# sohmandal/classpose

Hardware: AMD Instinct MI355X
Metric: wsi_tiles_per_sec (higher is better)
Workload: dtype bf16; 1 GPU; configs[1]: synthetic 10000x10000 WSI (1936 tiles), tile 256 / overlap 32, conic 7 classes, ViT-L ClassTransformer depth 24 random-init, batch 32 sub-tiles = 8 WSI tiles/step, every step a distinct batch of the rank's shard (tiles sharded k % n_gpus, at most 256 distinct batches resident, longer runs wrap) streamed pinned host -> hipMemcpyAsync inside the timed region (the reader decodes ahead int; slide=10000, tile=256, overlap=32, batch_subtiles=32, distinct_batches=143, records_gathered=2048, decode_ahead_batches_at_t0=4, device_resident_batches_at_t0=1

## Files before the change

### classpose_amd/csrc/cpx_net.hip

```cpp
#include "cpx_internal.h"
#include <algorithm>

typedef __attribute__((ext_vector_type(8))) __bf16 bf16x8;
typedef __attribute__((ext_vector_type(8))) _Float16 f16x8;
typedef __attribute__((ext_vector_type(16))) float f32x16;

template <bool F16>
__device__ __forceinline__ f32x16 mfma32(const uint4 &a, const uint4 &b, f32x16 c) {
    if constexpr (F16)
        return __builtin_amdgcn_mfma_f32_32x32x16_f16(*reinterpret_cast<const f16x8 *>(&a),
                                                      *reinterpret_cast<const f16x8 *>(&b), c, 0, 0, 0);
    else
        return __builtin_amdgcn_mfma_f32_32x32x16_bf16(*reinterpret_cast<const bf16x8 *>(&a),
                                                       *reinterpret_cast<const bf16x8 *>(&b), c, 0, 0, 0);
}
template <bool F16>
__device__ __forceinline__ unsigned short h_from_f32(float f) {
    if constexpr (F16) { _Float16 h = (_Float16)f; return *reinterpret_cast<unsigned short *>(&h); }
    else return f32_to_bf16(f);
}
template <bool F16>
__device__ __forceinline__ float f32_from_h(unsigned short u) {
    if constexpr (F16) return (float)*reinterpret_cast<_Float16 *>(&u);
    else return bf16_to_f32(u);
}

typedef __attribute__((ext_vector_type(2))) float f32x2_t;
typedef __attribute__((ext_vector_type(2))) __bf16 bf16x2_t;
typedef __attribute__((ext_vector_type(2))) _Float16 f16x2_t;
template <bool F16>
__device__ __forceinline__ unsigned pack2(float lo, float hi) {
    f32x2_t v = {lo, hi};
    if constexpr (F16) return __builtin_bit_cast(unsigned, __builtin_convertvector(v, f16x2_t));
    else return __builtin_bit_cast(unsigned, __builtin_convertvector(v, bf16x2_t));
}

template <int C, bool F16>
__global__ void __launch_bounds__(256) k_layernorm(const unsigned short *__restrict__ x,
                                                   const float *__restrict__ w,
                                                   const float *__restrict__ b, int rows, float eps,
                                                   unsigned short *__restrict__ out) {
    constexpr int PER = C / 64;
    const int lane = threadIdx.x & 63;
    const int row = blockIdx.x * 4 + (threadIdx.x >> 6);
    if (row >= rows) return;
    const unsigned short *xr = x + (size_t)row * C + lane * PER;
    float v[PER];
    if constexpr (PER == 16) {
        uint4 a = *reinterpret_cast<const uint4 *>(xr), c = *reinterpret_cast<const uint4 *>(xr + 8);
        unsigned u[8] = {a.x, a.y, a.z, a.w, c.x, c.y, c.z, c.w};
#pragma unroll
        for (int i = 0; i < 8; ++i) { v[2 * i] = f32_from_h<F16>(u[i] & 0xFFFF); v[2 * i + 1] = f32_from_h<F16>(u[i] >> 16); }
    } else {
        uint2 a = *reinterpret_cast<const uint2 *>(xr);
        v[0] = f32_from_h<F16>(a.x & 0xFFFF); v[1] = f32_from_h<F16>(a.x >> 16);
        v[2] = f32_from_h<F16>(a.y & 0xFFFF); v[3] = f32_from_h<F16>(a.y >> 16);
    }
    float s = 0.f;
#pragma unroll
    for (int i = 0; i < PER; ++i) s += v[i];
#pragma unroll
    for (int o = 32; o > 0; o >>= 1) s += __shfl_xor(s, o);
    const float mean = s * (1.0f / C);
    float q = 0.f;
#pragma unroll
    for (int i = 0; i < PER; ++i) { float d = v[i] - mean; q += d * d; }
#pragma unroll
    for (int o = 32; o > 0; o >>= 1) q += __shfl_xor(q, o);
    const float rstd = rsqrtf(q * (1.0f / C) + eps);
    unsigned short o16[PER];
#pragma unroll
    for (int i = 0; i < PER; ++i) {
        float y = (v[i] - mean) * rstd * w[lane * PER + i] + b[lane * PER + i];
        o16[i] = h_from_f32<F16>(y);
    }
    unsigned short *orow = out + (size_t)row * C + lane * PER;
    if constexpr (PER == 16) {
        uint4 a, c;
        a.x = o16[0] | (o16[1] << 16); a.y = o16[2] | (o16[3] << 16); a.z = o16[4] | (o16[5] << 16); a.w = o16[6] | (o16[7] << 16);
        c.x = o16[8] | (o16[9] << 16); c.y = o16[10] | (o16[11] << 16); c.z = o16[12] | (o16[13] << 16); c.w = o16[14] | (o16[15] << 16);
        *reinterpret_cast<uint4 *>(orow) = a;
        *reinterpret_cast<uint4 *>(orow + 8) = c;
    } else {
        uint2 a;
        a.x = o16[0] | (o16[1] << 16); a.y = o16[2] | (o16[3] << 16);
        *reinterpret_cast<uint2 *>(orow) = a;
    }
}

int cpx_layernorm_half(int dtype, const void *x, const float *w, const float *b, int rows, int C,
                       float eps, void *out, void *stream) {
    CPX_REQUIRE(x && w && b && out && rows > 0 && (C == 1024 || C == 256));
    CPX_REQUIRE(dtype == CPX_DT_BF16 || dtype == CPX_DT_F16);
    hipStream_t s = (hipStream_t)stream;
    dim3 grid(cpx_cdiv(rows, 4)), block(256);
    const bool f16 = dtype == CPX_DT_F16;
    if (C == 1024) {
        if (f16) hipLaunchKernelGGL((k_layernorm<1024, true>), grid, block, 0, s, (const unsigned short *)x, w, b, rows, eps, (unsigned short *)out);
        else hipLaunchKernelGGL((k_layernorm<1024, false>), grid, block, 0, s, (const unsigned short *)x, w, b, rows, eps, (unsigned short *)out);
    } else {
        if (f16) hipLaunchKernelGGL((k_layernorm<256, true>), grid, block, 0, s, (const unsigned short *)x, w, b, rows, eps, (unsigned short *)out);
        else hipLaunchKernelGGL((k_layernorm<256, false>), grid, block, 0, s, (const unsigned short *)x, w, b, rows, eps, (unsigned short *)out);
    }
    CPX_CHECK_LAUNCH();
    return CPX_OK;
}
extern "C" int cpx_layernorm(int dtype, const void *x, const float *w, const float *b, int rows, int C,
                             float eps, void *out, void *stream) {
    if (dtype == CPX_DT_F32) return cpx_layernorm_f32((const float *)x, w, b, rows, C, eps, (float *)out, stream);
    return cpx_layernorm_half(dtype, x, w, b, rows, C, eps, out, stream);
}
extern "C" int cpx_layernorm_bf16(const void *x, const float *w, const float *b, int rows, int C,
                                  float eps, void *out, void *stream) {
    return cpx_layernorm_half(CPX_DT_BF16, x, w, b, rows, C, eps, out, stream);
}

__global__ void __launch_bounds__(256) k_v_transpose(const unsigned short *__restrict__ qkv,
                                                     unsigned short *__restrict__ vT) {
    __shared__ unsigned short tile[64][66];
    const int t0 = blockIdx.x * 64, h = blockIdx.y, s = blockIdx.z;
    const int tid = threadIdx.x;
    {
        int tok = tid >> 2, c = (tid & 3) * 16;
        const unsigned short *src = qkv + ((size_t)s * 1024 + t0 + tok) * 3072 + 2048 + h * 64 + c;
        uint4 a = *reinterpret_cast<const uint4 *>(src), b = *reinterpret_cast<const uint4 *>(src + 8);
        unsigned u[8] = {a.x, a.y, a.z, a.w, b.x, b.y, b.z, b.w};
#pragma unroll
        for (int i = 0; i < 8; ++i) { tile[tok][c + 2 * i] = u[i] & 0xFFFF; tile[tok][c + 2 * i + 1] = u[i] >> 16; }
    }
    __syncthreads();
    {
        int d = tid >> 2, c = (tid & 3) * 16;
        unsigned u[8];
#pragma unroll
        for (int i = 0; i < 8; ++i) u[i] = tile[c + 2 * i][d] | ((unsigned)tile[c + 2 * i + 1][d] << 16);
        unsigned short *dst = vT + (((size_t)s * 16 + h) * 64 + d) * 1024 + t0 + c;
        *reinterpret_cast<uint4 *>(dst) = make_uint4(u[0], u[1], u[2], u[3]);
        *reinterpret_cast<uint4 *>(dst + 8) = make_uint4(u[4], u[5], u[6], u[7]);
    }
}

#define ATT_THREADS 256
__device__ __forceinline__ int pi_perm(int r) { return (r & ~12) | ((r & 4) << 1) | ((r & 8) >> 1); }

#define A4_SLOT 8192
#define A4_G_LD 66
#define A4_LDS_BYTES (4 * A4_SLOT + 4 * 32 * A4_G_LD * 2)
template <int OFF>
__device__ __forceinline__ uint4 a4_read128(unsigned addr) {
    uint4 v;
    asm volatile("ds_read_b128 %0, %1 offset:%2" : "=v"(v) : "v"(addr), "n"(OFF));
    return v;
}
template <bool F16>
__global__ void __launch_bounds__(ATT_THREADS, 3) k_attention4p(const unsigned short *__restrict__ qkv,
                                                                const unsigned short *__restrict__ vT,
                                                                const unsigned short *__restrict__ relh,
                                                                const unsigned short *__restrict__ relw,
                                                                unsigned short *__restrict__ out, int xcd_order) {
    extern __shared__ __attribute__((aligned(16))) char a4_smem[];
    const int tid = threadIdx.x, lane = tid & 63;
    const int wave = __builtin_amdgcn_readfirstlane(tid >> 6);
    const int r = lane & 31, h2 = lane >> 5;
    const int lin = (blockIdx.z * gridDim.y + blockIdx.y) * gridDim.x + blockIdx.x;
    int rg = blockIdx.x, head = blockIdx.y, s = blockIdx.z;
    if (xcd_order) {
        const int j = lin >> 3, pair = (j >> 3) * 8 + (lin & 7);
        rg = j & 7; head = pair & 15; s = pair >> 4;
    }
    const int qh = rg * 4 + wave;
    const size_t tok0 = (size_t)s * 1024;
    const int kkey = tid >> 3, vd = tid >> 2;
    const unsigned short *ksrc = qkv + (tok0 + kkey) * 3072 + 1024 + head * 64 + (((tid & 7) ^ ((kkey >> 1) & 7)) * 8);
    const unsigned short *vsrc = vT + (((size_t)s * 16 + head) * 64 + vd) * 1024 + (((tid & 3) ^ ((vd >> 2) & 3)) * 8);
    char *dma_dst = a4_smem + wave * 1024;
    auto issue = [&](int kh) {
        char *d = dma_dst + (kh & 3) * A4_SLOT;
        __builtin_amdgcn_global_load_lds((const __attribute__((address_space(1))) void *)(ksrc + (size_t)kh * 32 * 3072),
                                         (__attribute__((address_space(3))) void *)d, 16, 0, 0);
        __builtin_amdgcn_global_load_lds((const __attribute__((address_space(1))) void *)(vsrc + kh * 32),
                                         (__attribute__((address_space(3))) void *)(d + 4096), 16, 0, 0);
    };
    issue(0); issue(1); issue(2);

    const unsigned short *qrow = qkv + (tok0 + qh * 32 + r) * 3072 + head * 64;
    uint4 qf[4];
#pragma unroll
    for (int ks = 0; ks < 4; ++ks) qf[ks] = *reinterpret_cast<const uint4 *>(qrow + 16 * ks + 8 * h2);
    _Float16 *G = reinterpret_cast<_Float16 *>(a4_smem + 4 * A4_SLOT) + wave * 32 * A4_G_LD;
    auto compute_G = [&](const unsigned short *table) {
#pragma unroll
        for (int jb = 0; jb < 2; ++jb) {
            f32x16 acc;
#pragma unroll
            for (int i = 0; i < 16; ++i) acc[i] = 0.f;
#pragma unroll
            for (int ks = 0; ks < 4; ++ks) {
                uint4 tf = *reinterpret_cast<const uint4 *>(table + (jb * 32 + r) * 64 + 16 * ks + 8 * h2);
                acc = mfma32<F16>(tf, qf[ks], acc);
            }
#pragma unroll
            for (int i = 0; i < 16; ++i) G[r * A4_G_LD + jb * 32 + (i & 3) + 8 * (i >> 2) + 4 * h2] = (_Float16)acc[i];
        }
    };
    compute_G(relw);
    f32x16 GW;
#pragma unroll
    for (int i = 0; i < 16; ++i) GW[i] = (float)G[r * A4_G_LD + (r - pi_perm((i & 3) + 8 * (i >> 2) + 4 * h2) + 31)];
    compute_G(relh);
    asm volatile("s_waitcnt vmcnt(0) lgkmcnt(0)" ::: "memory");
    __builtin_amdgcn_s_barrier();

    const unsigned lds0 = (unsigned)(size_t)(__attribute__((address_space(3))) char *)a4_smem;
    const int krow = pi_perm(r);
    unsigned ka[4], va[4];
#pragma unroll
    for (int ks = 0; ks < 4; ++ks) ka[ks] = lds0 + (unsigned)(krow * 128 + (((2 * ks + h2) ^ ((krow >> 1) & 7)) * 16));
#pragma unroll
    for (int db = 0; db < 2; ++db)
#pragma unroll
        for (int st = 0; st < 2; ++st) {
            const int d = db * 32 + r;
            va[db * 2 + st] = lds0 + 4096u + (unsigned)(d * 64 + (((2 * st + h2) ^ ((d >> 2) & 3)) * 16));
        }
    const unsigned gaddr = lds0 + 4u * A4_SLOT + (unsigned)((wave * 32 * A4_G_LD + r * A4_G_LD + qh + 31) * 2);

    auto qk = [&](auto slot_tag) {
        constexpr int SL = decltype(slot_tag)::value;
        const uint4 k0 = a4_read128<SL * A4_SLOT>(ka[0]), k1 = a4_read128<SL * A4_SLOT>(ka[1]);
        const uint4 k2 = a4_read128<SL * A4_SLOT>(ka[2]), k3 = a4_read128<SL * A4_SLOT>(ka[3]);
        asm volatile("s_waitcnt lgkmcnt(0)" ::: "memory");
        __builtin_amdgcn_sched_barrier(0);
        f32x16 S = mfma32<F16>(k0, qf[0], GW);
        S = mfma32<F16>(k1, qf[1], S);
        S = mfma32<F16>(k2, qf[2], S);
        S = mfma32<F16>(k3, qf[3], S);
        return S;
    };
    using std::integral_constant;
    f32x16 S = qk(integral_constant<int, 0>{});
    f32x16 O0, O1;
#pragma unroll
    for (int i = 0; i < 16; ++i) { O0[i] = 0.f; O1[i] = 0.f; }
    float m_run = -1e30f, l_run = 0.f;
    const float cexp = 0.125f * 1.44269504088896340736f;
    constexpr float HEADROOM = F16 ? 3.0f : 6.0f;

    auto tile = [&](const int kh, auto slot_tag, auto next_tag, auto tail_tag) {
        constexpr int SL = decltype(slot_tag)::value, SN = decltype(next_tag)::value, TAIL = decltype(tail_tag)::value;
        if constexpr (TAIL < 2) asm volatile("s_waitcnt vmcnt(2)" ::: "memory");
        else asm volatile("s_waitcnt vmcnt(0)" ::: "memory");
        __builtin_amdgcn_s_barrier();
        if constexpr (TAIL == 0) issue(kh + 3);
        unsigned gh_bits;
        asm volatile("ds_read_u16 %0, %1" : "=v"(gh_bits) : "v"(gaddr - 2u * (unsigned)kh));
        f32x16 Sn = S;
        if constexpr (TAIL < 3) Sn = qk(integral_constant<int, SN>{});
        else {
            asm volatile("s_waitcnt lgkmcnt(0)" : "+v"(gh_bits)::"memory");
            __builtin_amdgcn_sched_barrier(0);
        }
        const float gh = (float)__builtin_bit_cast(_Float16, (unsigned short)gh_bits);
        float p[16];
        unsigned pk[8];
        {
            const float off = (gh - m_run) * cexp;
#pragma unroll
            for (int i = 0; i < 16; ++i) p[i] = __builtin_amdgcn_exp2f(__builtin_fmaf(S[i], cexp, off));
#pragma unroll
            for (int j = 0; j < 8; ++j) pk[j] = pack2<F16>(p[2 * j], p[2 * j + 1]);
        }
        const bool resc = __builtin_expect(__any(((pk[0] | pk[1] | pk[2]) | (pk[3] | pk[4] | pk[5]) | (pk[6] | pk[7])) & 0x40004000u), 0);
        if (resc) {
            float mx = __builtin_fmaxf(__builtin_fmaxf(S[0], S[1]), S[2]);
#pragma unroll
            for (int i = 3; i < 15; i += 2) mx = __builtin_fmaxf(__builtin_fmaxf(mx, S[i]), S[i + 1]);
            mx = __builtin_fmaxf(mx, S[15]);
            mx = __builtin_fmaxf(mx, __shfl_xor(mx, 32)) + gh + HEADROOM / cexp;
            const float m_new = __builtin_fmaxf(m_run, mx);
            const float alpha = __builtin_amdgcn_exp2f((m_run - m_new) * cexp);
            m_run = m_new;
            l_run *= alpha;
#pragma unroll
            for (int i = 0; i < 16; ++i) { O0[i] *= alpha; O1[i] *= alpha; }
            const float off = (gh - m_run) * cexp;
#pragma unroll
            for (int i = 0; i < 16; ++i) p[i] = __builtin_amdgcn_exp2f(__builtin_fmaf(S[i], cexp, off));
#pragma unroll
            for (int j = 0; j < 8; ++j) pk[j] = pack2<F16>(p[2 * j], p[2 * j + 1]);
        }
        const float a0 = (p[0] + p[1]) + (p[2] + p[3]), a1 = (p[4] + p[5]) + (p[6] + p[7]);
        const float a2 = (p[8] + p[9]) + (p[10] + p[11]), a3 = (p[12] + p[13]) + (p[14] + p[15]);
        l_run += (a0 + a1) + (a2 + a3);
        const uint4 pf0 = make_uint4(pk[0], pk[1], pk[2], pk[3]), pf1 = make_uint4(pk[4], pk[5], pk[6], pk[7]);
        const uint4 v00 = a4_read128<SL * A4_SLOT>(va[0]), v01 = a4_read128<SL * A4_SLOT>(va[1]);
        const uint4 v10 = a4_read128<SL * A4_SLOT>(va[2]), v11 = a4_read128<SL * A4_SLOT>(va[3]);
        asm volatile("s_waitcnt lgkmcnt(0)" ::: "memory");
        __builtin_amdgcn_sched_barrier(0);
        O0 = mfma32<F16>(v00, pf0, O0);
        O1 = mfma32<F16>(v10, pf0, O1);
        O0 = mfma32<F16>(v01, pf1, O0);
        O1 = mfma32<F16>(v11, pf1, O1);
        S = Sn;
    };
    using T0 = integral_constant<int, 0>;
    for (int kh0 = 0; kh0 < 28; kh0 += 4) {
        tile(kh0 + 0, integral_constant<int, 0>{}, integral_constant<int, 1>{}, T0{});
        tile(kh0 + 1, integral_constant<int, 1>{}, integral_constant<int, 2>{}, T0{});
        tile(kh0 + 2, integral_constant<int, 2>{}, integral_constant<int, 3>{}, T0{});
        tile(kh0 + 3, integral_constant<int, 3>{}, integral_constant<int, 0>{}, T0{});
    }
    tile(28, integral_constant<int, 0>{}, integral_constant<int, 1>{}, T0{});
    tile(29, integral_constant<int, 1>{}, integral_constant<int, 2>{}, integral_constant<int, 1>{});
    tile(30, integral_constant<int, 2>{}, integral_constant<int, 3>{}, integral_constant<int, 2>{});
    tile(31, integral_constant<int, 3>{}, integral_constant<int, 0>{}, integral_constant<int, 3>{});
    const float inv = 1.0f / (l_run + __shfl_xor(l_run, 32));
    unsigned short *orow = out + (tok0 + qh * 32 + r) * 1024 + head * 64;
#pragma unroll
    for (int db = 0; db < 2; ++db)
#pragma unroll
        for (int g4 = 0; g4 < 4; g4 += 2) {
            const f32x16 &O = db ? O1 : O0;
            unsigned ax = pack2<F16>(O[4 * g4 + 0] * inv, O[4 * g4 + 1] * inv), ay = pack2<F16>(O[4 * g4 + 2] * inv, O[4 * g4 + 3] * inv);
            unsigned bx = pack2<F16>(O[4 * g4 + 4] * inv, O[4 * g4 + 5] * inv), by = pack2<F16>(O[4 * g4 + 6] * inv, O[4 * g4 + 7] * inv);
            const auto rx = __builtin_amdgcn_permlane32_swap(ax, bx, false, false);
            const auto ry = __builtin_amdgcn_permlane32_swap(ay, by, false, false);
            *reinterpret_cast<uint4 *>(orow + db * 32 + 8 * g4 + 8 * h2) = make_uint4(rx[0], ry[0], rx[1], ry[1]);
        }
}

CPX_SWITCH(g_att_xcd, 1);
CPX_SWITCH(g_att_v8, 2);
#ifdef CPX_DEBUG
extern "C" void cpx_attention_set_variant(int v8) { g_att_v8 = v8; }
extern "C" void cpx_attention_set_xcd_order(int v) { g_att_xcd = v; }
#endif
extern "C" int cpx_attention_relpos(const void *qkv, const void *rel_h, const void *rel_w,
                                    int n_subtiles, void *vT_ws, void *out, void *stream) {
    return cpx_attention_half(CPX_DT_BF16, qkv, rel_h, rel_w, n_subtiles, vT_ws, out, stream, true);
}
extern "C" int cpx_attention(int dtype, const void *qkv, const void *rel_h, const void *rel_w,
                             int n_subtiles, void *vT_ws, void *out, void *stream) {
    if (dtype == CPX_DT_F32)
        return cpx_attention_f32((const float *)qkv, (const float *)rel_h, (const float *)rel_w, n_subtiles, (float *)out, stream);
    return cpx_attention_half(dtype, qkv, rel_h, rel_w, n_subtiles, vT_ws, out, stream, true);
}
int cpx_attention_half(int dtype, const void *qkv, const void *rel_h, const void *rel_w, int n_subtiles,
                       void *vT_ws, void *out, void *stream, bool transpose_v) {
    CPX_REQUIRE(qkv && rel_h && rel_w && vT_ws && out && n_subtiles > 0);
    CPX_REQUIRE(dtype == CPX_DT_BF16 || dtype == CPX_DT_F16);
#ifdef CPX_DEBUG
    CPX_REQUIRE(g_att_v8 == 2 || g_att_v8 == 7);
#endif
    hipStream_t s = (hipStream_t)stream;
    if (transpose_v)
        hipLaunchKernelGGL(k_v_transpose, dim3(16, 16, n_subtiles), dim3(256), 0, s,
                           (const unsigned short *)qkv, (unsigned short *)vT_ws);
#ifdef CPX_DEBUG
    if (g_att_v8 == 7) {
        const dim3 grid4(8, 16, n_subtiles);
        static CpxOncePerDevice once4;
        once4([] {
            (void)hipFuncSetAttribute((const void *)k_attention4p<true>, hipFuncAttributeMaxDynamicSharedMemorySize, A4_LDS_BYTES);
            (void)hipFuncSetAttribute((const void *)k_attention4p<false>, hipFuncAttributeMaxDynamicSharedMemorySize, A4_LDS_BYTES);
        });
        if (dtype == CPX_DT_F16)
            hipLaunchKernelGGL((k_attention4p<true>), grid4, dim3(ATT_THREADS), A4_LDS_BYTES, s, (const unsigned short *)qkv, (const unsigned short *)vT_ws,
                               (const unsigned short *)rel_h, (const unsigned short *)rel_w, (unsigned short *)out, g_att_xcd);
        else
            hipLaunchKernelGGL((k_attention4p<false>), grid4, dim3(ATT_THREADS), A4_LDS_BYTES, s, (const unsigned short *)qkv, (const unsigned short *)vT_ws,
                               (const unsigned short *)rel_h, (const unsigned short *)rel_w, (unsigned short *)out, g_att_xcd);
        CPX_CHECK_LAUNCH();
        return CPX_OK;
    }
#endif
    return cpx_attention2w_launch(dtype, qkv, vT_ws, rel_h, rel_w, n_subtiles, out, g_att_xcd, s);
}

struct NetWs {
    size_t off_x, off_xn, off_qkv, off_vt, off_ao, off_h, off_neck, off_neck2, off_st, total;
};
static NetWs net_ws(int nS) {
    NetWs w; size_t o = 0; const size_t M = (size_t)nS * 1024;
    auto take = [&](size_t b) { size_t r = o; o = cpx_align_up(o + b, 256); return r; };
    w.off_x = take(M * 1024 * 2);
    w.off_xn = take(M * 1024 * 2);
    w.off_qkv = take(M * 3072 * 2);
    w.off_vt = take(M * 1024 * 2);
    w.off_ao = take(M * 1024 * 2);
    w.off_h = take(M * 4096 * 2);
    w.off_neck = take(M * 256 * 2);
    w.off_neck2 = take(M * 256 * 2);
    w.off_st = take(M * 8 * sizeof(float));
    w.total = o;
    return w;
}
extern "C" size_t cpx_net_workspace_bytes(int n_subtiles, int dtype) {
    if (n_subtiles <= 0) return 0;
    return dtype == CPX_DT_F32 ? cpx_net_f32_workspace_bytes(n_subtiles) : net_ws(n_subtiles).total;
}

extern "C" size_t cpx_net_neck_offset(int n_subtiles, int dtype) {
    if (n_subtiles <= 0 || dtype < CPX_DT_BF16 || dtype > CPX_DT_F32) return 0;
    return dtype == CPX_DT_F32 ? cpx_net_f32_neck_offset(n_subtiles) : net_ws(n_subtiles).off_neck2;
}
// ... 326 lines not shown
```

### classpose_amd/csrc/cpx_pre.hip

```cpp
#include "cpx_common.h"

#define NTHR 256

__device__ __forceinline__ void cv_linear_tap(int d, double scale, int slen, bool clamp_weight,
                                              int &s0, int &s1, int &w0, int &w1) {
    float f = (float)(((double)d + 0.5) * scale - 0.5);
    int s = (int)floorf(f);
    f -= (float)s;
    if (clamp_weight) {
        if (s < 0) { f = 0.f; s = 0; }
        if (s >= slen - 1) { f = 0.f; s = slen - 1; }
    }
    w0 = __float2int_rn((1.f - f) * 2048.f);
    w1 = __float2int_rn(f * 2048.f);
    s0 = min(max(s, 0), slen - 1);
    s1 = min(max(s + 1, 0), slen - 1);
}

__global__ void k_resize_linear_u8(const uint8_t *__restrict__ src, int sh, int sw,
                                   uint8_t *__restrict__ dst, int dh, int dw, double scale_x,
                                   double scale_y, int area2) {
    int p = blockIdx.x * NTHR + threadIdx.x;
    if (p >= dh * dw) return;
    int dy = p / dw, dx = p - dy * dw;
    const uint8_t *s = src + (size_t)blockIdx.y * sh * sw * 3;
    uint8_t *o = dst + ((size_t)blockIdx.y * dh * dw + p) * 3;
    if (area2) {
        const uint8_t *r0 = s + ((size_t)(2 * dy) * sw + 2 * dx) * 3, *r1 = r0 + (size_t)sw * 3;
        for (int c = 0; c < 3; ++c) o[c] = (uint8_t)((r0[c] + r0[3 + c] + r1[c] + r1[3 + c] + 2) >> 2);
        return;
    }
    int x0, x1, a0, a1, y0, y1, b0, b1;
    cv_linear_tap(dx, scale_x, sw, true, x0, x1, a0, a1);
    cv_linear_tap(dy, scale_y, sh, false, y0, y1, b0, b1);
    const uint8_t *r0 = s + (size_t)y0 * sw * 3, *r1 = s + (size_t)y1 * sw * 3;
    for (int c = 0; c < 3; ++c) {
        int h0 = r0[x0 * 3 + c] * a0 + r0[x1 * 3 + c] * a1;
        int h1 = r1[x0 * 3 + c] * a0 + r1[x1 * 3 + c] * a1;
        o[c] = (uint8_t)((((b0 * (h0 >> 4)) >> 16) + ((b1 * (h1 >> 4)) >> 16) + 2) >> 2);
    }
}

extern "C" int cpx_resize_linear_u8(const uint8_t *src, int nT, int sh, int sw, uint8_t *dst, int dh,
                                    int dw, void *stream) {
    CPX_REQUIRE(src && dst && nT > 0 && sh > 0 && sw > 0 && dh > 0 && dw > 0);
    CPX_REQUIRE((long long)dh * dw < (1ll << 31) && (long long)sh * sw < (1ll << 31));
    hipStream_t s = (hipStream_t)stream;
    if (sh == dh && sw == dw) {
        hipError_t e = hipMemcpyAsync(dst, src, (size_t)nT * sh * sw * 3, hipMemcpyDeviceToDevice, s);
        CPX_REQUIRE(e == hipSuccess);
        return CPX_OK;
    }
    double scale_x = 1.0 / ((double)dw / (double)sw), scale_y = 1.0 / ((double)dh / (double)sh);
    int area2 = (sw == 2 * dw && sh == 2 * dh) ? 1 : 0;
    hipLaunchKernelGGL(k_resize_linear_u8, dim3(cpx_cdiv((long long)dh * dw, NTHR), nT), dim3(NTHR), 0, s,
                       src, sh, sw, dst, dh, dw, scale_x, scale_y, area2);
    CPX_CHECK_LAUNCH();
    return CPX_OK;
}

__global__ void k_hist_u8(const uint8_t *__restrict__ tiles, int HW, uint32_t *__restrict__ hist) {
    __shared__ uint32_t sh[3 * 256];
    for (int i = threadIdx.x; i < 768; i += NTHR) sh[i] = 0;
    __syncthreads();
    const uint8_t *t = tiles + (size_t)blockIdx.y * HW * 3;
    for (int p = (blockIdx.x * NTHR + threadIdx.x) * 4; p < HW; p += gridDim.x * NTHR * 4) {
        int n = min(4, HW - p);
        for (int k = 0; k < n; ++k) {
            const uint8_t *px = t + (size_t)(p + k) * 3;
            atomicAdd(&sh[px[0]], 1u);
            atomicAdd(&sh[256 + px[1]], 1u);
            atomicAdd(&sh[512 + px[2]], 1u);
        }
    }
    __syncthreads();
    uint32_t *h = hist + (size_t)blockIdx.y * 768;
    for (int i = threadIdx.x; i < 768; i += NTHR)
        if (sh[i]) atomicAdd(&h[i], sh[i]);
}

__device__ __forceinline__ float np_lerp(float a, float b, float t) {
    float diff = b - a;
    float r = a + diff * t;
    if (t >= 0.5f) r = b - diff * (1.0f - t);
    return r;
}
__global__ void k_norm_stats(const uint32_t *__restrict__ hist, int nTC, int HW, int lo_prev,
                             float lo_g, int hi_prev, float hi_g, float *__restrict__ stats) {
    const int lane = threadIdx.x & 63;
    const int tc = (blockIdx.x * blockDim.x + threadIdx.x) >> 6;
    if (tc >= nTC) return;
    const uint4 c = *reinterpret_cast<const uint4 *>(hist + (size_t)tc * 256 + 4 * lane);
    const long long s0 = c.x, s1 = s0 + c.y, s2 = s1 + c.z, s3 = s2 + c.w;
    long long incl = s3;
#pragma unroll
    for (int o = 1; o < 64; o <<= 1) {
        const long long up = __shfl_up(incl, o);
        if (lane >= o) incl += up;
    }
    const long long excl = incl - s3;
    auto value_at = [&](int k) -> float {
        const unsigned long long m = __ballot(incl > (long long)k);
        const int l = __ffsll((long long)m) - 1;
        int v = 0;
        if (lane == l) v = 4 * lane + (excl + s0 > k ? 0 : (excl + s1 > k ? 1 : (excl + s2 > k ? 2 : 3)));
        return (float)__shfl(v, l);
    };
    const float g0 = value_at(lo_prev), g1 = value_at(min(lo_prev + 1, HW - 1));
    const float g2 = value_at(hi_prev), g3 = value_at(min(hi_prev + 1, HW - 1));
    const unsigned long long nz = __ballot(s3 > 0);
    const int lmin = __ffsll((long long)nz) - 1, lmax = 63 - __clzll((long long)nz);
    int vlo = 0, vhi = 0;
    if (lane == lmin) vlo = 4 * lane + (c.x ? 0 : (c.y ? 1 : (c.z ? 2 : 3)));
    if (lane == lmax) vhi = 4 * lane + (c.w ? 3 : (c.z ? 2 : (c.y ? 1 : 0)));
    const int vmin = __shfl(vlo, lmin), vmax = __shfl(vhi, lmax);
    if (lane != 0) return;
    float x01 = np_lerp(g0, g1, lo_g);
    float x99 = np_lerp(g2, g3, hi_g);
    float den = x99 - x01;
    float mode;
    if (vmax == vmin) mode = 0.f;
    else if (den > (float)1e-3) mode = 1.f;
    else mode = 2.f;
    stats[tc * 4 + 0] = x01;
    stats[tc * 4 + 1] = den;
    stats[tc * 4 + 2] = mode;
    stats[tc * 4 + 3] = x99;
}

__device__ __forceinline__ float norm_px(uint8_t v, const float *st) {
    float x = (float)v;
    float mode = st[2];
    if (mode == 1.f) { x = x - st[0]; x = __fdiv_rn(x, st[1]); }
    else if (mode == 2.f) x = 0.f;
    return x;
}

__global__ void k_norm_apply(const uint8_t *__restrict__ tiles, const float *__restrict__ stats,
                             int HW, float *__restrict__ out) {
    int i = blockIdx.x * NTHR + threadIdx.x;
    if (i >= HW * 3) return;
    size_t t = blockIdx.y;
    int c = i % 3;
    out[t * HW * 3 + i] = norm_px(tiles[t * HW * 3 + i], stats + (t * 3 + c) * 4);
}

extern "C" int cpx_normalize_stats_u8(const uint8_t *tiles, int nT, int H, int W, int lo_prev,
                                      float lo_gamma, int hi_prev, float hi_gamma, float *stats,
                                      uint32_t *hist_ws, void *stream) {
    CPX_REQUIRE(tiles && stats && hist_ws && nT > 0 && H > 0 && W > 0);
    CPX_REQUIRE(lo_prev >= 0 && hi_prev >= lo_prev && hi_prev < H * W);
    hipStream_t s = (hipStream_t)stream;
    CPX_HIP(hipMemsetAsync(hist_ws, 0, sizeof(uint32_t) * 768 * (size_t)nT, s));
    int nb = min(64, cpx_cdiv((long long)H * W, NTHR * 4));
    hipLaunchKernelGGL(k_hist_u8, dim3(nb, nT), dim3(NTHR), 0, s, tiles, H * W, hist_ws);
    hipLaunchKernelGGL(k_norm_stats, dim3(cpx_cdiv(nT * 3, 4)), dim3(256), 0, s, hist_ws, nT * 3,
                       H * W, lo_prev, lo_gamma, hi_prev, hi_gamma, stats);
    CPX_CHECK_LAUNCH();
    return CPX_OK;
}

extern "C" int cpx_normalize_apply_u8(const uint8_t *tiles, const float *stats, int nT, int H, int W,
                                      float *out, void *stream) {
    CPX_REQUIRE(tiles && stats && out && nT > 0 && H > 0 && W > 0);
    hipLaunchKernelGGL(k_norm_apply, dim3(cpx_cdiv((long long)H * W * 3, NTHR), nT), dim3(NTHR), 0,
                       (hipStream_t)stream, tiles, stats, H * W, out);
    CPX_CHECK_LAUNCH();
    return CPX_OK;
}

struct TilingDev {
    int H, W, ypad1, xpad1, Ly, Lx, ny, nx, b, augment;
    int ys[16], xs[16];
};
static int tiling_to_dev(const cpx_tiling *t, TilingDev *d) {
    CPX_REQUIRE(t && t->ny >= 1 && t->nx >= 1 && t->ny <= 16 && t->nx <= 16);
    CPX_REQUIRE(t->bsize > 0 && t->bsize % 8 == 0);
    d->H = t->H; d->W = t->W; d->ypad1 = t->ypad1; d->xpad1 = t->xpad1; d->Ly = t->Ly; d->Lx = t->Lx;
    d->ny = t->ny; d->nx = t->nx; d->b = t->bsize; d->augment = t->augment;
    for (int i = 0; i < 16; ++i) { d->ys[i] = t->ystart[i]; d->xs[i] = t->xstart[i]; }
    return CPX_OK;
}

__device__ __forceinline__ float padded_px(const uint8_t *tiles, const float *stats, const TilingDev &g,
                                           size_t t, int Yp, int Xp, int c) {
    int Y = Yp - g.ypad1, X = Xp - g.xpad1;
    if ((unsigned)Y >= (unsigned)g.H || (unsigned)X >= (unsigned)g.W) return 0.f;
    return norm_px(tiles[(t * g.H * g.W + (size_t)Y * g.W + X) * 3 + c], stats + (t * 3 + c) * 4);
}

__device__ __forceinline__ unsigned short f32_to_f16(float f) {
    _Float16 h = (_Float16)f;
    return *reinterpret_cast<unsigned short *>(&h);
}
template <int DT>
__global__ void k_make_patches(const uint8_t *__restrict__ tiles, const float *__restrict__ stats,
                               TilingDev g, void *__restrict__ patches_v) {
    const int tok_per = (g.b / 8) * (g.b / 8);
    const int per_sub = tok_per * 24;
    int i = blockIdx.x * NTHR + threadIdx.x;
    if (i >= per_sub) return;
    int sub = blockIdx.y;
    int t = sub / (g.ny * g.nx), ji = sub - t * g.ny * g.nx;
    int j = ji / g.nx, ii_t = ji - j * g.nx;
    int tok = i / 24, r = i - tok * 24;
    int c = r >> 3, ii = r & 7;
    int ph = tok / (g.b / 8), pw = tok - ph * (g.b / 8);
    bool fy = g.augment && (ii_t & 1) && !(j & 1);
    bool fx = g.augment && (j & 1) && !(ii_t & 1);
    if (g.augment && (j & 1) && (ii_t & 1)) { fy = true; fx = true; }
    int y = 8 * ph + ii;
    int sy = fy ? g.b - 1 - y : y;
    union { unsigned short h[8]; uint4 v; } o;
    float f[8];
#pragma unroll
    for (int jj = 0; jj < 8; ++jj) {
        int x = 8 * pw + jj;
        int sx = fx ? g.b - 1 - x : x;
        float v = padded_px(tiles, stats, g, t, g.ys[j] + sy, g.xs[ii_t] + sx, c);
        f[jj] = v;
        o.h[jj] = DT == 1 ? f32_to_f16(v) : f32_to_bf16(v);
    }
    const size_t e = ((size_t)sub * tok_per + tok) * 192 + c * 64 + ii * 8;
    if constexpr (DT == 2) {
        float *patches = (float *)patches_v;
        *reinterpret_cast<float4 *>(patches + e) = make_float4(f[0], f[1], f[2], f[3]);
        *reinterpret_cast<float4 *>(patches + e + 4) = make_float4(f[4], f[5], f[6], f[7]);
    } else {
        *reinterpret_cast<uint4 *>((unsigned short *)patches_v + e) = o.v;
    }
}

__global__ void k_make_subtiles_f32(const uint8_t *__restrict__ tiles, const float *__restrict__ stats,
                                    TilingDev g, float *__restrict__ out) {
    int i = blockIdx.x * NTHR + threadIdx.x;
    int per = 3 * g.b * g.b;
    if (i >= per) return;
    int sub = blockIdx.y;
    int t = sub / (g.ny * g.nx), ji = sub - t * g.ny * g.nx;
    int j = ji / g.nx, ii_t = ji - j * g.nx;
    int c = i / (g.b * g.b), r = i - c * g.b * g.b;
    int y = r / g.b, x = r - y * g.b;
    bool fy = g.augment && (ii_t & 1) && !(j & 1);
    bool fx = g.augment && (j & 1) && !(ii_t & 1);
    if (g.augment && (j & 1) && (ii_t & 1)) { fy = true; fx = true; }
    int sy = fy ? g.b - 1 - y : y, sx = fx ? g.b - 1 - x : x;
    out[(size_t)sub * per + i] = padded_px(tiles, stats, g, t, g.ys[j] + sy, g.xs[ii_t] + sx, c);
}

extern "C" int cpx_make_patches(const uint8_t *tiles, const float *stats, int nT,
                                const cpx_tiling *tiling, int dtype, void *patches, void *stream) {
    TilingDev g; int rc = tiling_to_dev(tiling, &g); if (rc) return rc;
    CPX_REQUIRE(tiles && stats && patches && nT > 0 && dtype >= 0 && dtype <= 2);
    int per_sub = (g.b / 8) * (g.b / 8) * 24;
    const dim3 grid(cpx_cdiv(per_sub, NTHR), nT * g.ny * g.nx);
    if (dtype == 2) hipLaunchKernelGGL(k_make_patches<2>, grid, dim3(NTHR), 0, (hipStream_t)stream, tiles, stats, g, patches);
    else if (dtype == 1) hipLaunchKernelGGL(k_make_patches<1>, grid, dim3(NTHR), 0, (hipStream_t)stream, tiles, stats, g, patches);
    else hipLaunchKernelGGL(k_make_patches<0>, grid, dim3(NTHR), 0, (hipStream_t)stream, tiles, stats, g, patches);
    CPX_CHECK_LAUNCH();
    return CPX_OK;
}
extern "C" int cpx_make_subtiles(const uint8_t *tiles, const float *stats, int nT,
                                 const cpx_tiling *tiling, void *patches, void *stream) {
    return cpx_make_patches(tiles, stats, nT, tiling, 0, patches, stream);
}

extern "C" int cpx_make_subtiles_f32(const uint8_t *tiles, const float *stats, int nT,
                                     const cpx_tiling *tiling, float *subtiles, void *stream) {
    TilingDev g; int rc = tiling_to_dev(tiling, &g); if (rc) return rc;
    CPX_REQUIRE(tiles && stats && subtiles && nT > 0);
    hipLaunchKernelGGL(k_make_subtiles_f32, dim3(cpx_cdiv(3 * g.b * g.b, NTHR), nT * g.ny * g.nx),
                       dim3(NTHR), 0, (hipStream_t)stream, tiles, stats, g, subtiles);
    CPX_CHECK_LAUNCH();
    return CPX_OK;
}

template <bool TOKEN_MAJOR>
__global__ void k_blend(const float *__restrict__ src, const float *__restrict__ src2, int ld, int ncls,
                        TilingDev g, const double *__restrict__ taper, float *__restrict__ dP,
                        float *__restrict__ cellprob, float *__restrict__ logits) {
    int idx = blockIdx.x * NTHR + threadIdx.x;
    const int HW = g.H * g.W;
    if (idx >= HW) return;
    const int ch = blockIdx.z;
    size_t t = blockIdx.y;
    int Y = idx / g.W, X = idx - Y * g.W;
    int Yp = Y + g.ypad1, Xp = X + g.xpad1;
    const int tb = g.b / 8;
    float acc = 0.f;
    double navg = 0.0;
    for (int j = 0; j < g.ny; ++j) {
        int y = Yp - g.ys[j];
        if ((unsigned)y >= (unsigned)g.b) continue;
        for (int i = 0; i < g.nx; ++i) {
            int x = Xp - g.xs[i];
            if ((unsigned)x >= (unsigned)g.b) continue;
            bool fy = g.augment && (i & 1) && !(j & 1);
            bool fx = g.augment && (j & 1) && !(i & 1);
            if (g.augment && (j & 1) && (i & 1)) { fy = true; fx = true; }
            int sy = fy ? g.b - 1 - y : y, sx = fx ? g.b - 1 - x : x;
            size_t sub = (t * g.ny + j) * g.nx + i;
            float v;
            if (TOKEN_MAJOR) {
                int tok = (sy >> 3) * tb + (sx >> 3);
                int col = (ch < 3 ? ch * 64 : 192 + (ch - 3) * 64) + (sy & 7) * 8 + (sx & 7);
                v = src[(sub * tb * tb + tok) * (size_t)ld + col];
            } else {
                v = ch < 3 ? src[((sub * 3 + ch) * g.b + sy) * (size_t)g.b + sx]
                           : src2[((sub * ncls + (ch - 3)) * g.b + sy) * (size_t)g.b + sx];
            }
            if ((ch == 0 && fy) || (ch == 1 && fx)) v = -v;
            double m = taper[x] * taper[y];
            acc = (float)((double)acc + (double)v * m);
            navg = navg + m;
        }
    }
    float r = (float)((double)acc / navg);
    if (ch < 2) dP[(t * 2 + ch) * HW + idx] = r;
    else if (ch == 2) cellprob[t * HW + idx] = r;
    else logits[(t * ncls + (ch - 3)) * HW + idx] = r;
}

extern "C" int cpx_blend_subtiles(const float *head, int ld_head, int ncls, int nT,
                                  const cpx_tiling *tiling, const double *taper1d, float *dP,
                                  float *cellprob, float *logits, void *stream) {
    TilingDev g; int rc = tiling_to_dev(tiling, &g); if (rc) return rc;
    CPX_REQUIRE(head && taper1d && dP && cellprob && nT > 0 && ncls >= 0 && (ncls == 0 || logits));
    CPX_REQUIRE(ld_head >= 192 + ncls * 64);
    hipLaunchKernelGGL(k_blend<true>, dim3(cpx_cdiv(g.H * g.W, NTHR), nT, 3 + ncls), dim3(NTHR), 0,
                       (hipStream_t)stream, head, (const float *)nullptr, ld_head, ncls, g, taper1d,
                       dP, cellprob, logits);
    CPX_CHECK_LAUNCH();
    return CPX_OK;
}

extern "C" int cpx_blend_subtiles_nchw(const float *y, const float *y_class, int ncls, int nT,
                                       const cpx_tiling *tiling, const double *taper1d, float *dP,
                                       float *cellprob, float *logits, void *stream) {
    TilingDev g; int rc = tiling_to_dev(tiling, &g); if (rc) return rc;
    CPX_REQUIRE(y && taper1d && dP && cellprob && nT > 0 && ncls >= 0 && (ncls == 0 || (logits && y_class)));
    hipLaunchKernelGGL(k_blend<false>, dim3(cpx_cdiv(g.H * g.W, NTHR), nT, 3 + ncls), dim3(NTHR), 0,
                       (hipStream_t)stream, y, y_class, 0, ncls, g, taper1d, dP, cellprob, logits);
    CPX_CHECK_LAUNCH();
    return CPX_OK;
}
```

Baseline: 372.6 tiles/s.

## Rework preprocessing, layernorm-256, histogram/stats and blend kernels for fewer passes

Adds a dedicated C=256 layernorm kernel that uses 32 lanes per row, handling eight rows per block. Fuses the histogram and normalisation-stats kernels into one launch with replicated shared histograms, which removes the memset and the second launch. Makes patch extraction load 24 contiguous bytes per thread and produce all three channels at once. Replaces the token-major blend with a row kernel that gathers 4 pixels and up to 10 channels per thread using vector loads and stores. These changes cut launches and memory traffic in pre- and post-processing, but change the reduction order, and the blend kernel now carries more register pressure.

```diff
diff --git a/classpose_amd/csrc/cpx_net.hip b/classpose_amd/csrc/cpx_net.hip
--- a/classpose_amd/csrc/cpx_net.hip
+++ b/classpose_amd/csrc/cpx_net.hip
@@ -88,6 +88,46 @@
     }
 }
 
+template <bool F16>
+__global__ void __launch_bounds__(256) k_layernorm256(const unsigned short *__restrict__ x, const float *__restrict__ w,
+                                                      const float *__restrict__ b, int rows, float eps,
+                                                      unsigned short *__restrict__ out) {
+#pragma clang fp contract(off)
+    constexpr int C = 256;
+    const int sub = threadIdx.x & 31;
+    const int row = blockIdx.x * 8 + (threadIdx.x >> 5);
+    if (row >= rows) return;
+    const uint4 a = *reinterpret_cast<const uint4 *>(x + (size_t)row * C + sub * 8);
+    const unsigned u[4] = {a.x, a.y, a.z, a.w};
+    float v[8];
+#pragma unroll
+    for (int i = 0; i < 4; ++i) { v[2 * i] = f32_from_h<F16>(u[i] & 0xFFFF); v[2 * i + 1] = f32_from_h<F16>(u[i] >> 16); }
+    float s0 = 0.f, s1 = 0.f;
+#pragma unroll
+    for (int i = 0; i < 4; ++i) { s0 += v[i]; s1 += v[4 + i]; }
+#pragma unroll
+    for (int o = 16; o > 0; o >>= 1) { s0 += __shfl_xor(s0, o); s1 += __shfl_xor(s1, o); }
+    const float mean = (s0 + s1) * (1.0f / C);
+    float d[8];
+#pragma unroll
+    for (int i = 0; i < 8; ++i) d[i] = v[i] - mean;
+    float q0 = d[0] * d[0], q1 = d[4] * d[4];
+#pragma unroll
+    for (int i = 1; i < 4; ++i) { q0 += d[i] * d[i]; q1 += d[4 + i] * d[4 + i]; }
+#pragma unroll
+    for (int o = 16; o > 0; o >>= 1) { q0 += __shfl_xor(q0, o); q1 += __shfl_xor(q1, o); }
+    const float rstd = rsqrtf(__builtin_fmaf(q0 + q1, 1.0f / C, eps));
+    unsigned short o16[8];
+#pragma unroll
+    for (int i = 0; i < 8; ++i) {
+        float y = __builtin_fmaf(d[i] * rstd, w[sub * 8 + i], b[sub * 8 + i]);
+        o16[i] = h_from_f32<F16>(y);
+    }
+    uint4 r;
+    r.x = o16[0] | (o16[1] << 16); r.y = o16[2] | (o16[3] << 16); r.z = o16[4] | (o16[5] << 16); r.w = o16[6] | (o16[7] << 16);
+    *reinterpret_cast<uint4 *>(out + (size_t)row * C + sub * 8) = r;
+}
+
 int cpx_layernorm_half(int dtype, const void *x, const float *w, const float *b, int rows, int C,
                        float eps, void *out, void *stream) {
     CPX_REQUIRE(x && w && b && out && rows > 0 && (C == 1024 || C == 256));
@@ -99,8 +139,9 @@
         if (f16) hipLaunchKernelGGL((k_layernorm<1024, true>), grid, block, 0, s, (const unsigned short *)x, w, b, rows, eps, (unsigned short *)out);
         else hipLaunchKernelGGL((k_layernorm<1024, false>), grid, block, 0, s, (const unsigned short *)x, w, b, rows, eps, (unsigned short *)out);
     } else {
-        if (f16) hipLaunchKernelGGL((k_layernorm<256, true>), grid, block, 0, s, (const unsigned short *)x, w, b, rows, eps, (unsigned short *)out);
-        else hipLaunchKernelGGL((k_layernorm<256, false>), grid, block, 0, s, (const unsigned short *)x, w, b, rows, eps, (unsigned short *)out);
+        const dim3 grid8(cpx_cdiv(rows, 8));
+        if (f16) hipLaunchKernelGGL((k_layernorm256<true>), grid8, block, 0, s, (const unsigned short *)x, w, b, rows, eps, (unsigned short *)out);
+        else hipLaunchKernelGGL((k_layernorm256<false>), grid8, block, 0, s, (const unsigned short *)x, w, b, rows, eps, (unsigned short *)out);
     }
     CPX_CHECK_LAUNCH();
     return CPX_OK;
diff --git a/classpose_amd/csrc/cpx_pre.hip b/classpose_amd/csrc/cpx_pre.hip
--- a/classpose_amd/csrc/cpx_pre.hip
+++ b/classpose_amd/csrc/cpx_pre.hip
@@ -59,38 +59,14 @@
     return CPX_OK;
 }
 
-__global__ void k_hist_u8(const uint8_t *__restrict__ tiles, int HW, uint32_t *__restrict__ hist) {
-    __shared__ uint32_t sh[3 * 256];
-    for (int i = threadIdx.x; i < 768; i += NTHR) sh[i] = 0;
-    __syncthreads();
-    const uint8_t *t = tiles + (size_t)blockIdx.y * HW * 3;
-    for (int p = (blockIdx.x * NTHR + threadIdx.x) * 4; p < HW; p += gridDim.x * NTHR * 4) {
-        int n = min(4, HW - p);
-        for (int k = 0; k < n; ++k) {
-            const uint8_t *px = t + (size_t)(p + k) * 3;
-            atomicAdd(&sh[px[0]], 1u);
-            atomicAdd(&sh[256 + px[1]], 1u);
-            atomicAdd(&sh[512 + px[2]], 1u);
-        }
-    }
-    __syncthreads();
-    uint32_t *h = hist + (size_t)blockIdx.y * 768;
-    for (int i = threadIdx.x; i < 768; i += NTHR)
-        if (sh[i]) atomicAdd(&h[i], sh[i]);
-}
-
 __device__ __forceinline__ float np_lerp(float a, float b, float t) {
     float diff = b - a;
     float r = a + diff * t;
     if (t >= 0.5f) r = b - diff * (1.0f - t);
     return r;
 }
-__global__ void k_norm_stats(const uint32_t *__restrict__ hist, int nTC, int HW, int lo_prev,
-                             float lo_g, int hi_prev, float hi_g, float *__restrict__ stats) {
-    const int lane = threadIdx.x & 63;
-    const int tc = (blockIdx.x * blockDim.x + threadIdx.x) >> 6;
-    if (tc >= nTC) return;
-    const uint4 c = *reinterpret_cast<const uint4 *>(hist + (size_t)tc * 256 + 4 * lane);
+__device__ __forceinline__ void norm_stats_wave(const uint4 c, int lane, int tc, int HW, int lo_prev, float lo_g,
+                                                int hi_prev, float hi_g, float *__restrict__ stats) {
     const long long s0 = c.x, s1 = s0 + c.y, s2 = s1 + c.z, s3 = s2 + c.w;
     long long incl = s3;
 #pragma unroll
@@ -128,6 +104,53 @@
     stats[tc * 4 + 3] = x99;
 }
 
+#define HIST_THR 1024
+#define HIST_COPIES 32
+template <int C>
+__device__ __forceinline__ void hist_add16(const uint4 &a, const uint4 &b, const uint4 &d, uint32_t *mine) {
+    const uint32_t w[12] = {a.x, a.y, a.z, a.w, b.x, b.y, b.z, b.w, d.x, d.y, d.z, d.w};
+#pragma unroll
+    for (int k = 0; k < 16; ++k) {
+        const int byte = 3 * k + C;
+        atomicAdd(&mine[((w[byte >> 2] >> ((byte & 3) * 8)) & 255u) * HIST_COPIES], 1u);
+    }
+}
+
+__global__ void __launch_bounds__(HIST_THR) k_hist_stats_u8(const uint8_t *__restrict__ tiles, int HW, int lo_prev,
+                                                            float lo_g, int hi_prev, float hi_g,
+                                                            float *__restrict__ stats, uint32_t *__restrict__ hist) {
+    __shared__ uint32_t sh[256 * HIST_COPIES];
+    __shared__ __attribute__((aligned(16))) uint32_t tot[256];
+    const int tc = blockIdx.x, t = tc / 3, c = tc - 3 * t;
+    for (int i = threadIdx.x; i < 256 * HIST_COPIES; i += HIST_THR) sh[i] = 0;
+    __syncthreads();
+    const uint8_t *p = tiles + (size_t)t * HW * 3;
+    uint32_t *mine = sh + (threadIdx.x & (HIST_COPIES - 1));
+    const int ngrp = ((uintptr_t)p & 15) ? 0 : HW / 16;
+    for (int gi = threadIdx.x; gi < ngrp; gi += HIST_THR) {
+        const uint4 *q = reinterpret_cast<const uint4 *>(p + (size_t)gi * 48);
+        const uint4 a = q[0], b = q[1], d = q[2];
+        if (c == 0) hist_add16<0>(a, b, d, mine);
+        else if (c == 1) hist_add16<1>(a, b, d, mine);
+        else hist_add16<2>(a, b, d, mine);
+    }
+    for (int px = ngrp * 16 + threadIdx.x; px < HW; px += HIST_THR)
+        atomicAdd(&mine[p[(size_t)px * 3 + c] * HIST_COPIES], 1u);
+    __syncthreads();
+    if (threadIdx.x < 256) {
+        uint32_t s = 0;
+#pragma unroll
+        for (int r = 0; r < HIST_COPIES; ++r)
+            s += sh[threadIdx.x * HIST_COPIES + ((r + threadIdx.x) & (HIST_COPIES - 1))];
+        tot[threadIdx.x] = s;
+        hist[(size_t)tc * 256 + threadIdx.x] = s;
+    }
+    __syncthreads();
+    if (threadIdx.x < 64)
+        norm_stats_wave(*reinterpret_cast<const uint4 *>(tot + 4 * threadIdx.x), threadIdx.x, tc, HW, lo_prev, lo_g,
+                        hi_prev, hi_g, stats);
+}
+
 __device__ __forceinline__ float norm_px(uint8_t v, const float *st) {
     float x = (float)v;
     float mode = st[2];
@@ -151,11 +174,8 @@
     CPX_REQUIRE(tiles && stats && hist_ws && nT > 0 && H > 0 && W > 0);
     CPX_REQUIRE(lo_prev >= 0 && hi_prev >= lo_prev && hi_prev < H * W);
     hipStream_t s = (hipStream_t)stream;
-    CPX_HIP(hipMemsetAsync(hist_ws, 0, sizeof(uint32_t) * 768 * (size_t)nT, s));
-    int nb = min(64, cpx_cdiv((long long)H * W, NTHR * 4));
-    hipLaunchKernelGGL(k_hist_u8, dim3(nb, nT), dim3(NTHR), 0, s, tiles, H * W, hist_ws);
-    hipLaunchKernelGGL(k_norm_stats, dim3(cpx_cdiv(nT * 3, 4)), dim3(256), 0, s, hist_ws, nT * 3,
-                       H * W, lo_prev, lo_gamma, hi_prev, hi_gamma, stats);
+    hipLaunchKernelGGL(k_hist_stats_u8, dim3(nT * 3), dim3(HIST_THR), 0, s, tiles, H * W, lo_prev, lo_gamma,
+                       hi_prev, hi_gamma, stats, hist_ws);
     CPX_CHECK_LAUNCH();
     return CPX_OK;
 }
@@ -197,37 +217,69 @@
 __global__ void k_make_patches(const uint8_t *__restrict__ tiles, const float *__restrict__ stats,
                                TilingDev g, void *__restrict__ patches_v) {
     const int tok_per = (g.b / 8) * (g.b / 8);
-    const int per_sub = tok_per * 24;
+    const int per_sub = tok_per * 8;
     int i = blockIdx.x * NTHR + threadIdx.x;
     if (i >= per_sub) return;
     int sub = blockIdx.y;
     int t = sub / (g.ny * g.nx), ji = sub - t * g.ny * g.nx;
     int j = ji / g.nx, ii_t = ji - j * g.nx;
-    int tok = i / 24, r = i - tok * 24;
-    int c = r >> 3, ii = r & 7;
+    int tok = i >> 3, ii = i & 7;
     int ph = tok / (g.b / 8), pw = tok - ph * (g.b / 8);
     bool fy = g.augment && (ii_t & 1) && !(j & 1);
     bool fx = g.augment && (j & 1) && !(ii_t & 1);
     if (g.augment && (j & 1) && (ii_t & 1)) { fy = true; fx = true; }
     int y = 8 * ph + ii;
     int sy = fy ? g.b - 1 - y : y;
-    union { unsigned short h[8]; uint4 v; } o;
-    float f[8];
-#pragma unroll
-    for (int jj = 0; jj < 8; ++jj) {
-        int x = 8 * pw + jj;
-        int sx = fx ? g.b - 1 - x : x;
-        float v = padded_px(tiles, stats, g, t, g.ys[j] + sy, g.xs[ii_t] + sx, c);
-        f[jj] = v;
-        o.h[jj] = DT == 1 ? f32_to_f16(v) : f32_to_bf16(v);
-    }
-    const size_t e = ((size_t)sub * tok_per + tok) * 192 + c * 64 + ii * 8;
-    if constexpr (DT == 2) {
-        float *patches = (float *)patches_v;
-        *reinterpret_cast<float4 *>(patches + e) = make_float4(f[0], f[1], f[2], f[3]);
-        *reinterpret_cast<float4 *>(patches + e + 4) = make_float4(f[4], f[5], f[6], f[7]);
+    const int Y = g.ys[j] + sy - g.ypad1;
+    const int Xa = g.xs[ii_t] + (fx ? g.b - 8 - 8 * pw : 8 * pw) - g.xpad1;
+    float f[3][8];
+    if ((unsigned)Y < (unsigned)g.H && Xa >= 0 && Xa + 8 <= g.W) {
+        const uint8_t *p = tiles + (((size_t)t * g.H + Y) * g.W + Xa) * 3;
+        uint32_t w[6];
+        if (((uintptr_t)p & 7) == 0) {
+            const uint2 a = reinterpret_cast<const uint2 *>(p)[0], b = reinterpret_cast<const uint2 *>(p)[1],
+                        d = reinterpret_cast<const uint2 *>(p)[2];
+            w[0] = a.x; w[1] = a.y; w[2] = b.x; w[3] = b.y; w[4] = d.x; w[5] = d.y;
+        } else {
+#pragma unroll
+            for (int k = 0; k < 6; ++k)
+                w[k] = p[4 * k] | (p[4 * k + 1] << 8) | (p[4 * k + 2] << 16) | ((uint32_t)p[4 * k + 3] << 24);
+        }
+#pragma unroll
+        for (int c = 0; c < 3; ++c) {
+            const float *st = stats + ((size_t)t * 3 + c) * 4;
+            float n[8];
+#pragma unroll
+            for (int k = 0; k < 8; ++k) {
+                const int byte = 3 * k + c;
+                n[k] = norm_px((uint8_t)((w[byte >> 2] >> ((byte & 3) * 8)) & 255u), st);
+            }
+#pragma unroll
+            for (int jj = 0; jj < 8; ++jj) f[c][jj] = fx ? n[7 - jj] : n[jj];
+        }
     } else {
-        *reinterpret_cast<uint4 *>((unsigned short *)patches_v + e) = o.v;
+#pragma unroll
+        for (int c = 0; c < 3; ++c)
+#pragma unroll
+            for (int jj = 0; jj < 8; ++jj) {
+                int x = 8 * pw + jj;
+                int sx = fx ? g.b - 1 - x : x;
+                f[c][jj] = padded_px(tiles, stats, g, t, g.ys[j] + sy, g.xs[ii_t] + sx, c);
+            }
+    }
+#pragma unroll
+    for (int c = 0; c < 3; ++c) {
+        const size_t e = ((size_t)sub * tok_per + tok) * 192 + c * 64 + ii * 8;
+        if constexpr (DT == 2) {
+            float *patches = (float *)patches_v;
+            *reinterpret_cast<float4 *>(patches + e) = make_float4(f[c][0], f[c][1], f[c][2], f[c][3]);
+            *reinterpret_cast<float4 *>(patches + e + 4) = make_float4(f[c][4], f[c][5], f[c][6], f[c][7]);
+        } else {
+            union { unsigned short h[8]; uint4 v; } o;
+#pragma unroll
+            for (int jj = 0; jj < 8; ++jj) o.h[jj] = DT == 1 ? f32_to_f16(f[c][jj]) : f32_to_bf16(f[c][jj]);
+            *reinterpret_cast<uint4 *>((unsigned short *)patches_v + e) = o.v;
+        }
     }
 }
 
@@ -252,7 +304,7 @@
                                 const cpx_tiling *tiling, int dtype, void *patches, void *stream) {
     TilingDev g; int rc = tiling_to_dev(tiling, &g); if (rc) return rc;
     CPX_REQUIRE(tiles && stats && patches && nT > 0 && dtype >= 0 && dtype <= 2);
-    int per_sub = (g.b / 8) * (g.b / 8) * 24;
+    int per_sub = (g.b / 8) * (g.b / 8) * 8;
     const dim3 grid(cpx_cdiv(per_sub, NTHR), nT * g.ny * g.nx);
     if (dtype == 2) hipLaunchKernelGGL(k_make_patches<2>, grid, dim3(NTHR), 0, (hipStream_t)stream, tiles, stats, g, patches);
     else if (dtype == 1) hipLaunchKernelGGL(k_make_patches<1>, grid, dim3(NTHR), 0, (hipStream_t)stream, tiles, stats, g, patches);
@@ -275,8 +327,7 @@
     return CPX_OK;
 }
 
-template <bool TOKEN_MAJOR>
-__global__ void k_blend(const float *__restrict__ src, const float *__restrict__ src2, int ld, int ncls,
+__global__ void k_blend(const float *__restrict__ src, const float *__restrict__ src2, int ncls,
                         TilingDev g, const double *__restrict__ taper, float *__restrict__ dP,
                         float *__restrict__ cellprob, float *__restrict__ logits) {
     int idx = blockIdx.x * NTHR + threadIdx.x;
@@ -286,7 +337,6 @@
     size_t t = blockIdx.y;
     int Y = idx / g.W, X = idx - Y * g.W;
     int Yp = Y + g.ypad1, Xp = X + g.xpad1;
-    const int tb = g.b / 8;
     float acc = 0.f;
     double navg = 0.0;
     for (int j = 0; j < g.ny; ++j) {
@@ -300,15 +350,8 @@
             if (g.augment && (j & 1) && (i & 1)) { fy = true; fx = true; }
             int sy = fy ? g.b - 1 - y : y, sx = fx ? g.b - 1 - x : x;
             size_t sub = (t * g.ny + j) * g.nx + i;
-            float v;
-            if (TOKEN_MAJOR) {
-                int tok = (sy >> 3) * tb + (sx >> 3);
-                int col = (ch < 3 ? ch * 64 : 192 + (ch - 3) * 64) + (sy & 7) * 8 + (sx & 7);
-                v = src[(sub * tb * tb + tok) * (size_t)ld + col];
-            } else {
-                v = ch < 3 ? src[((sub * 3 + ch) * g.b + sy) * (size_t)g.b + sx]
-                           : src2[((sub * ncls + (ch - 3)) * g.b + sy) * (size_t)g.b + sx];
-            }
+            float v = ch < 3 ? src[((sub * 3 + ch) * g.b + sy) * (size_t)g.b + sx]
+                             : src2[((sub * ncls + (ch - 3)) * g.b + sy) * (size_t)g.b + sx];
             if ((ch == 0 && fy) || (ch == 1 && fx)) v = -v;
             double m = taper[x] * taper[y];
             acc = (float)((double)acc + (double)v * m);
@@ -319,6 +362,99 @@
     if (ch < 2) dP[(t * 2 + ch) * HW + idx] = r;
     else if (ch == 2) cellprob[t * HW + idx] = r;
     else logits[(t * ncls + (ch - 3)) * HW + idx] = r;
+}
+
+#define BLEND_CH 10
+__global__ void __launch_bounds__(NTHR) k_blend_rows(const float *__restrict__ src, int ld, int nch, TilingDev g,
+                                                     const double *__restrict__ taper, float *__restrict__ dP,
+                                                     float *__restrict__ cellprob, float *__restrict__ logits,
+                                                     int vec_in, int vec_out) {
+    const int lane = threadIdx.x & 63, wv = threadIdx.x >> 6;
+    const int X0 = (blockIdx.x * (NTHR / 64) + wv) * 32 + (lane >> 4) * 8 + (lane & 1) * 4;
+    const int Y = blockIdx.y * 8 + ((lane >> 1) & 7);
+    if (Y >= g.H || X0 >= g.W) return;
+    const size_t t = blockIdx.z;
+    const int HW = g.H * g.W, tb = g.b / 8, ncls = nch - 3;
+    const int Yp = Y + g.ypad1, Xp0 = X0 + g.xpad1;
+    const int npx = min(4, g.W - X0);
+    for (int c0 = 0; c0 < nch; c0 += BLEND_CH) {
+        float acc[BLEND_CH][4];
+        double navg[4] = {0.0, 0.0, 0.0, 0.0};
+#pragma unroll
+        for (int c = 0; c < BLEND_CH; ++c)
+#pragma unroll
+            for (int k = 0; k < 4; ++k) acc[c][k] = 0.f;
+        for (int j = 0; j < g.ny; ++j) {
+            const int y = Yp - g.ys[j];
+            if ((unsigned)y >= (unsigned)g.b) continue;
+            const double ty = taper[y];
+            for (int i = 0; i < g.nx; ++i) {
+                const int x0 = Xp0 - g.xs[i];
+                if (x0 + npx <= 0 || x0 >= g.b) continue;
+                bool fy = g.augment && (i & 1) && !(j & 1);
+                bool fx = g.augment && (j & 1) && !(i & 1);
+                if (g.augment && (j & 1) && (i & 1)) { fy = true; fx = true; }
+                const int sy = fy ? g.b - 1 - y : y;
+                const size_t sub = (t * g.ny + j) * g.nx + i;
+                const float *rowp = src + (sub * tb * tb + (size_t)(sy >> 3) * tb) * (size_t)ld + (sy & 7) * 8;
+                bool ok[4];
+                double m[4];
+#pragma unroll
+                for (int k = 0; k < 4; ++k) {
+                    ok[k] = k < npx && (unsigned)(x0 + k) < (unsigned)g.b;
+                    m[k] = 0.0;
+                    if (ok[k]) { m[k] = taper[x0 + k] * ty; navg[k] = navg[k] + m[k]; }
+                }
+                if (vec_in && !(x0 & 3) && ok[0] && ok[3]) {
+                    const int sx = fx ? g.b - 4 - x0 : x0;
+                    const float *p = rowp + (size_t)(sx >> 3) * ld + (sx & 7);
+#pragma unroll
+                    for (int c = 0; c < BLEND_CH; ++c) {
+                        const int ch = c0 + c;
+                        if (ch >= nch) break;
+                        const float4 q = *reinterpret_cast<const float4 *>(p + ch * 64);
+                        float v[4] = {fx ? q.w : q.x, fx ? q.z : q.y, fx ? q.y : q.z, fx ? q.x : q.w};
+                        const bool neg = (ch == 0 && fy) || (ch == 1 && fx);
+#pragma unroll
+                        for (int k = 0; k < 4; ++k) {
+                            if (neg) v[k] = -v[k];
+                            acc[c][k] = (float)((double)acc[c][k] + (double)v[k] * m[k]);
+                        }
+                    }
+                } else {
+#pragma unroll
+                    for (int k = 0; k < 4; ++k) {
+                        if (!ok[k]) continue;
+                        const int sx = fx ? g.b - 1 - (x0 + k) : x0 + k;
+                        const float *p = rowp + (size_t)(sx >> 3) * ld + (sx & 7);
+#pragma unroll
+                        for (int c = 0; c < BLEND_CH; ++c) {
+                            const int ch = c0 + c;
+                            if (ch >= nch) break;
+                            float v = p[ch * 64];
+                            if ((ch == 0 && fy) || (ch == 1 && fx)) v = -v;
+                            acc[c][k] = (float)((double)acc[c][k] + (double)v * m[k]);
+                        }
+                    }
+                }
+            }
+        }
+        const int idx = Y * g.W + X0;
+#pragma unroll
+        for (int c = 0; c < BLEND_CH; ++c) {
+            const int ch = c0 + c;
+            if (ch >= nch) break;
+            float *o = ch < 2 ? dP + (t * 2 + ch) * HW : ch == 2 ? cellprob + t * HW : logits + (t * ncls + (ch - 3)) * HW;
+            float r[4];
+#pragma unroll
+            for (int k = 0; k < 4; ++k) r[k] = (float)((double)acc[c][k] / navg[k]);
+            if (vec_out) *reinterpret_cast<float4 *>(o + idx) = make_float4(r[0], r[1], r[2], r[3]);
+            else
+#pragma unroll
+                for (int k = 0; k < 4; ++k)
+                    if (k < npx) o[idx + k] = r[k];
+        }
+    }
 }
 
 extern "C" int cpx_blend_subtiles(const float *head, int ld_head, int ncls, int nT,
@@ -327,9 +463,11 @@
     TilingDev g; int rc = tiling_to_dev(tiling, &g); if (rc) return rc;
     CPX_REQUIRE(head && taper1d && dP && cellprob && nT > 0 && ncls >= 0 && (ncls == 0 || logits));
     CPX_REQUIRE(ld_head >= 192 + ncls * 64);
-    hipLaunchKernelGGL(k_blend<true>, dim3(cpx_cdiv(g.H * g.W, NTHR), nT, 3 + ncls), dim3(NTHR), 0,
-                       (hipStream_t)stream, head, (const float *)nullptr, ld_head, ncls, g, taper1d,
-                       dP, cellprob, logits);
+    const int vec_in = ld_head % 4 == 0 && (uintptr_t)head % 16 == 0;
+    const int vec_out = g.W % 4 == 0 && (uintptr_t)dP % 16 == 0 && (uintptr_t)cellprob % 16 == 0 &&
+                        (uintptr_t)logits % 16 == 0;
+    hipLaunchKernelGGL(k_blend_rows, dim3(cpx_cdiv(g.W, 32 * (NTHR / 64)), cpx_cdiv(g.H, 8), nT), dim3(NTHR), 0,
+                       (hipStream_t)stream, head, ld_head, 3 + ncls, g, taper1d, dP, cellprob, logits, vec_in, vec_out);
     CPX_CHECK_LAUNCH();
     return CPX_OK;
 }
@@ -339,8 +477,8 @@
                                        float *cellprob, float *logits, void *stream) {
     TilingDev g; int rc = tiling_to_dev(tiling, &g); if (rc) return rc;
     CPX_REQUIRE(y && taper1d && dP && cellprob && nT > 0 && ncls >= 0 && (ncls == 0 || (logits && y_class)));
-    hipLaunchKernelGGL(k_blend<false>, dim3(cpx_cdiv(g.H * g.W, NTHR), nT, 3 + ncls), dim3(NTHR), 0,
-                       (hipStream_t)stream, y, y_class, 0, ncls, g, taper1d, dP, cellprob, logits);
-    CPX_CHECK_LAUNCH();
-    return CPX_OK;
-}
+    hipLaunchKernelGGL(k_blend, dim3(cpx_cdiv(g.H * g.W, NTHR), nT, 3 + ncls), dim3(NTHR), 0,
+                       (hipStream_t)stream, y, y_class, ncls, g, taper1d, dP, cellprob, logits);
+    CPX_CHECK_LAUNCH();
+    return CPX_OK;
+}
```

Result: no change. 373.4 tiles/s (median of 6 runs) (+0.2%).
